# KleistLab/ADAPTed

Hardware: AMD Instinct MI355X
Metric: reads/sec (adapter+polyA detect), RNA004 200k-sample reads (higher is better)
Workload: dtype f32 samples/statistics, f64 cumulative sums + LLR trace

## Files before the change

adapted_amd/csrc/adapted_hip.hip:

```cpp
#include <hip/hip_runtime.h>

#include <cmath>
#include <cstdio>
#include <cstring>
#include <cstdlib>
#include <string>
#include <vector>

#include "adapted_hip.h"
#include "handle.h"
#include "common.h"
__device__ unsigned long long g_dbg[ADP_NDBG] = {0};
__device__ unsigned long long g_bs_tally[ADP_NTALLY][8] = {{0}};
#include "llr_stream.h"
#include "n1_select.h"
#include "n1_fused.h"
#include "peaks.h"
#include "synth.h"
#include "validate.h"
#include "cand_stats2.h"
#include "series_pipe.h"
#include "cnn_topk.h"
#include "cnn_conv.h"
#include "cnn_conv_split.h"
// ... 483 lines not shown
        hipLaunchKernelGGL((k_n1_pick<1, N1_SAMPLE>), pg, dim3(256), 0, st, mbs, gh, gb, gc, mode, thr);
        { Scope s(h, !profile ? nullptr : (mode ? "k_n1_hist<1> mad" : "k_n1_hist<1> med"));
          hipLaunchKernelGGL((k_n1_hist<1, SIG>), hg, dim3(N1_THREADS), 0, st, dsig, n, m, T, minibatch, mode, mbs, gh, gb, gc, 1, N1_ALWAYS, cb, collect, 1, 8, tails); }
        hipLaunchKernelGGL((k_n1_pick<1, N1_FULL>), pg, dim3(256), 0, st, mbs, gh, gb, gc, mode, thr);
        hipLaunchKernelGGL(k_n1_finish, pg, dim3(1024), 0, st, mbs, cb, gc, gb, mode, thr);
        hipLaunchKernelGGL((k_n1_hist<0, SIG>), hg, dim3(N1_THREADS), 0, st, dsig, n, m, T, minibatch, mode, mbs, gh, gb, gc, 1, N1_IF_BAD, cb, 0, 1, 8, tails);
        hipLaunchKernelGGL((k_n1_pick<0, N1_FALLBACK>), pg, dim3(256), 0, st, mbs, gh, gb, gc, mode, thr);
        hipLaunchKernelGGL((k_n1_hist<1, SIG>), hg, dim3(N1_THREADS), 0, st, dsig, n, m, T, minibatch, mode, mbs, gh, gb, gc, 1, N1_IF_BAD, cb, 0, 1, 8, tails);
        hipLaunchKernelGGL((k_n1_pick<1, N1_FALLBACK>), pg, dim3(256), 0, st, mbs, gh, gb, gc, mode, thr);
        { Scope s(h, !profile ? nullptr : (mode ? "k_n1_hist<2> mad" : "k_n1_hist<2> med"));
          hipLaunchKernelGGL((k_n1_hist<2, SIG>), hg, dim3(N1_THREADS), 0, st, dsig, n, m, T, minibatch, mode, mbs, gh, gb, gc, 1, N1_IF_NOT_DONE, cb, 0, 1, 8, tails); }
        hipLaunchKernelGGL((k_n1_pick<2, N1_FULL>), pg, dim3(256), 0, st, mbs, gh, gb, gc, mode, thr);
    }
    return 0;
}

struct PhaseSync {
    hipEvent_t wait[3] = {nullptr, nullptr, nullptr};
    hipEvent_t done[3] = {nullptr, nullptr, nullptr};
};

static __device__ __host__ inline SigF32 sig_from(const SigF32 &s, size_t r0, int m) { return SigF32{s.base + r0 * (size_t)m}; }
static __device__ __host__ inline SigI16 sig_from(const SigI16 &s, size_t r0, int m) { return SigI16{s.base + r0 * (size_t)m, s.scale + r0, s.offset + r0, s.full_len + r0}; }
static inline SigIdx sig_subset(const SigF32 &s, const int32_t *sel) { return SigIdx{s.base, sel}; }
static inline SigIdxI16 sig_subset(const SigI16 &s, const int32_t *sel) { return SigIdxI16{s.base, s.scale, s.offset, s.full_len, sel}; }

static void launch_cumsum(adp_handle *h, int n)
{
    const int split = env_int("ADP_CUMSUM_GATHER", 1) != 0;
    hipLaunchKernelGGL(k_cumsum, dim3((n + 63) / 64), dim3(64), 0, h->stream, h->down.as<float>(), h->nvalid.as<int32_t>(), h->Lp, n,
                       h->nck, h->ck.as<double2>(), h->tail.as<double2>(), split);
    if (split)
        hipLaunchKernelGGL(k_cumsum_gather, dim3((n + 63) / 64), dim3(64), 0, h->stream, h->down.as<float>(), h->nvalid.as<int32_t>(), h->Lp, n,
                           h->nck, h->ck.as<double2>(), h->tail.as<double2>());
}

static void launch_polya_peak(adp_handle *h, int n, int mbsize, const double *pkv)
{
    const int grid = n < h->pslots ? n : h->pslots;
    hipLaunchKernelGGL(k_polya_peak, dim3(grid), dim3(64), (size_t)(((h->Lp / 2 + 1) + 8) / 16 + 2) * 4, h->stream, h->trace.as<double>(), h->nvalid.as<int32_t>(), h->Lp,
                       h->bmax.as<double>(), h->bmin.as<double>(), h->nsum, h->adapter_idx.as<int32_t>(), n, mbsize, h->mbs.as<MbState>(),
                       h->pk.as<int32_t>(), h->mk.as<uint32_t>(), h->polya_idx.as<int32_t>(), h->npk.as<int32_t>(), pkv, env_int("ADP_PK_PREFIX", PK_PREFIX));
}

template <class SIG>
static int llr_enqueue(adp_handle *h, SIG dsig, const int32_t *dlen, int n, int m, int minibatch, int flags,
                       adp_row *rows_dev, int rows_kind , int32_t *mb_status_dev, double *mb_params_dev,
                       int upto, const PhaseSync *ps)
{
    int rc = 0;
    const int n_mb = (n + minibatch - 1) / minibatch;
    h->last_n = n; h->last_nmb = n_mb;
    ALLOCCHK(h->mbs.ensure((size_t)n_mb * sizeof(MbState)) || h->ghist.ensure((size_t)n_mb * N1_BINS * 4) || h->gbelow.ensure((size_t)n_mb * 8) || h->gcnt.ensure((size_t)n_mb * 8 * N1_NCNT));
    rc = alloc_all(h, n, true);
    if (rc) return rc;
    hipStream_t st = h->stream;
#ifdef ADP_ABLATE
    sync_ablate(h);
#endif
    if (ps && ps->wait[0]) HIPCHK(hipStreamWaitEvent(st, ps->wait[0], 0));
    MbState *mbs = h->mbs.as<MbState>();
    HIPCHK(hipMemsetAsync(mbs, 0, (size_t)n_mb * sizeof(MbState), st));
    HIPCHK(hipMemsetAsync(h->ghist.p, 0, (size_t)n_mb * N1_BINS * 4, st));
    HIPCHK(hipMemsetAsync(h->gbelow.p, 0, (size_t)n_mb * 8, st));
    HIPCHK(hipMemsetAsync(h->gcnt.p, 0, (size_t)n_mb * 8 * N1_NCNT, st));
    const int T = h->T;
    bool sp_forked = false, sp_done = false;
    if (h->L <= 0) {
        hipLaunchKernelGGL(k_mb_set_status, dim3((n_mb + 255) / 256), dim3(256), 0, st, mbs, n_mb, ADP_MB_EMPTY_TRACE);
        if (ps) for (int k = 0; k < 2; k++) { if (k && ps->wait[k]) HIPCHK(hipStreamWaitEvent(st, ps->wait[k], 0)); if (ps->done[k]) HIPCHK(hipEventRecord(ps->done[k], st)); }
    } else {
        const int32_t *tails = (flags & ADP_TAILS_NAN) ? dlen : nullptr;
        rc = launch_n1(h, dsig, n, m, T, minibatch, n_mb, true, tails);
        if (rc) return rc;
        const bool sp_fused = upto >= 8 && (flags & ADP_WITH_START_PEAK) && h->layout == ADP_LAYOUT_MINIBATCH &&
                              h->cfg.sp_downscale_factor == h->ds && h->off % h->ds == 0 && T > h->off && env_int("ADP_SP_FUSED", 1) != 0;
        if (sp_fused) {
            ALLOCCHK(h->sphead.ensure((size_t)n * sizeof(SpHead)));
            Scope s(h, "k_sp_head");
            hipLaunchKernelGGL(k_sp_head<SIG>, dim3(n), dim3(64), (size_t)64 * h->cfg.sp_downscale_factor * 4, st, dsig, dlen, n, m, h->cfg, h->off, h->sphead.as<SpHead>());
        }
        if (upto >= 2 && sp_fused) {
            { Scope s(h, "k_norm_pool");
              auto kern = (h->ds == 10 && std::is_same<SIG, SigF32>::value && env_int("ADP_NP_PREFETCH", 1)) ? k_norm_pool<SIG, true, 5> : k_norm_pool<SIG, true, 0>;
              hipLaunchKernelGGL(kern, dim3(n), dim3(256), (size_t)NP_TILE * h->ds * 4, st, dsig, m, T, h->off, h->ds, h->L, h->Lp,
                                 minibatch, mbs, h->down.as<float>(), h->nvalid.as<int32_t>(), (const int64_t *)nullptr,
                                 dlen, (flags & ADP_TAILS_NAN) ? 1 : 0, h->sphead.as<SpHead>(), (float)h->cfg.open_pore_pa); }
            const int cov0 = h->off / h->ds, cov1 = cov0 + (T - h->off) / h->ds;
            Scope s(h, "k_sp_tail");
            hipLaunchKernelGGL(k_sp_tail<SIG>, dim3(n), dim3(64), (size_t)64 * h->cfg.sp_downscale_factor * 4, st, dsig, dlen, n, m, h->cfg, cov0, cov1,
                               (const SpHead *)h->sphead.as<SpHead>(), h->sp.as<SpOut>());
            sp_done = true;
        } else if (upto >= 2) {
            Scope s(h, "k_norm_pool");
            const int64_t *rng = nullptr;
            if (h->layout == ADP_LAYOUT_SINGLE_READ) {
                ALLOCCHK(h->rng0.ensure((size_t)n * 16));
                std::vector<int64_t> hr((size_t)2 * n);
                for (int i = 0; i < n; i++) { hr[2 * i] = 0; hr[2 * i + 1] = T; }
                HIPCHK(hipMemcpyAsync(h->rng0.p, hr.data(), (size_t)n * 16, hipMemcpyHostToDevice, st));
                HIPCHK(hipStreamSynchronize(st));
                rng = h->rng0.as<int64_t>();
            }
            auto kern = (h->ds == 10 && !rng && std::is_same<SIG, SigF32>::value && env_int("ADP_NP_PREFETCH", 1)) ? k_norm_pool<SIG, false, 5> : k_norm_pool<SIG, false, 0>;
            hipLaunchKernelGGL(kern, dim3(n), dim3(256), (size_t)NP_TILE * h->ds * 4, st, dsig, m, T, h->off, h->ds, h->L, h->Lp,
                               minibatch, mbs, h->down.as<float>(), h->nvalid.as<int32_t>(), rng,
                               dlen, (flags & ADP_TAILS_NAN) ? 1 : 0, (SpHead *)nullptr, 0.f);
        }
        if (upto >= 2)
            hipLaunchKernelGGL(k_check_empty, dim3((n + 255) / 256), dim3(256), 0, st, h->nvalid.as<int32_t>(), n, minibatch, mbs);
        if (ps && ps->done[0]) HIPCHK(hipEventRecord(ps->done[0], st));
        if (upto >= 8 && (flags & ADP_WITH_START_PEAK) && !sp_fused) {
            HIPCHK(hipEventRecord(h->ev_fork, st));
            HIPCHK(hipStreamWaitEvent(h->stream2, h->ev_fork, 0));
            { Scope s(h, "k_start_peak", h->stream2);
              hipLaunchKernelGGL(k_start_peak<SIG>, dim3(n), dim3(64), (size_t)64 * h->cfg.sp_downscale_factor * 4, h->stream2, dsig, dlen, n, m, h->cfg, h->sp.as<SpOut>()); }
            HIPCHK(hipEventRecord(h->ev_join, h->stream2));
            sp_forked = true;
        }
        if (ps && ps->wait[1]) HIPCHK(hipStreamWaitEvent(st, ps->wait[1], 0));
        if (upto >= 3) {
            Scope s(h, "k_cumsum");
            launch_cumsum(h, n);
        }
        if (upto >= 4) {
            Scope s(h, "k_gains<1>");
            hipLaunchKernelGGL(k_gains<1>, dim3((n + GAINS_WPB - 1) / GAINS_WPB), dim3(64 * GAINS_WPB), 0, st, h->down.as<float>(), h->nvalid.as<int32_t>(), h->Lp, h->nck,
                               h->ck.as<double2>(), h->tail.as<double2>(), h->adapter_idx.as<int32_t>(), minibatch, mbs,
                               h->trace.as<double>(), h->bmax.as<double>(), h->bmin.as<double>(), h->nsum, h->t1.as<int2>(), 0, h->pk.as<int32_t>(), h->npk.as<int32_t>(), h->Lp / 2 + 1, h->gstat.as<double>(), n, h->oh1);
        }
        if (upto >= 5) {
            Scope s(h, "k_adapter_peak");
            hipLaunchKernelGGL(k_adapter_peak, dim3(n), dim3(64), 0, st, h->trace.as<double>(), h->nvalid.as<int32_t>(), h->Lp,
                               h->bmax.as<double>(), h->bmin.as<double>(), h->nsum, h->t1.as<int2>(), minibatch, mbs,
                               h->cfg.adapter_peak_prominence, h->cfg.adapter_peak_rel_height,
                               h->cfg.adapter_peak_width / h->ds, h->adapter_idx.as<int32_t>(), h->gstat.as<double>());
        }
        double *pkvp = (env_int("ADP_PK_VALUES", 1) && h->pkv.cap >= (size_t)n * (h->Lp / 2 + 1) * 8) ? h->pkv.as<double>() : nullptr;
        if (upto >= 6) {
            Scope s(h, "k_gains<2>");
            hipLaunchKernelGGL(k_gains<2>, dim3((n + GAINS_WPB - 1) / GAINS_WPB), dim3(64 * GAINS_WPB), 0, st, h->down.as<float>(), h->nvalid.as<int32_t>(), h->Lp, h->nck,
                               h->ck.as<double2>(), h->tail.as<double2>(), h->adapter_idx.as<int32_t>(), minibatch, mbs,
                               h->trace.as<double>(), h->bmax.as<double>(), h->bmin.as<double>(), h->nsum, h->t1.as<int2>(), 0, h->pk.as<int32_t>(), h->npk.as<int32_t>(), h->Lp / 2 + 1, h->gstat.as<double>(), n, 5, pkvp);
        }
        if (upto >= 7) {
            Scope s(h, "k_polya_peak");
            launch_polya_peak(h, n, minibatch, pkvp);
        }
        if (ps && ps->done[1]) HIPCHK(hipEventRecord(ps->done[1], st));
    }
    if (upto >= 8) {
        if (ps && ps->wait[2]) HIPCHK(hipStreamWaitEvent(st, ps->wait[2], 0));
        if (h->L > 0)
            hipLaunchKernelGGL(k_llr_bounds, dim3((n + 255) / 256), dim3(256), 0, st, h->adapter_idx.as<int32_t>(),
                               h->polya_idx.as<int32_t>(), n, h->ds, h->pos_off, h->bounds.as<int64_t>(), h->topk_none.as<int8_t>(), h->layout == ADP_LAYOUT_SINGLE_READ ? 1 : 0);
        rc = launch_validate(h, dsig, dlen, n, m, 1, minibatch, true);
        if (rc) return rc;
        if (flags & ADP_WITH_START_PEAK) {
            if (sp_forked) HIPCHK(hipStreamWaitEvent(st, h->ev_join, 0));
            else if (!sp_done) {
                Scope s(h, "k_start_peak");
                hipLaunchKernelGGL(k_start_peak<SIG>, dim3(n), dim3(64), (size_t)64 * h->cfg.sp_downscale_factor * 4, st, dsig, dlen, n, m, h->cfg, h->sp.as<SpOut>());
            }
            hipLaunchKernelGGL(k_sp_decorate, dim3((n + 255) / 256), dim3(256), 0, st, h->sp.as<SpOut>(), h->rows.as<adp_row>(), n, 0,
                               (const int32_t *)nullptr);
        }
        if (rows_dev)
            HIPCHK(hipMemcpyAsync(rows_dev, h->rows.p, (size_t)n * sizeof(adp_row), (hipMemcpyKind)rows_kind, st));
    }
    if (mb_status_dev)
        hipLaunchKernelGGL(k_mb_status_out, dim3((n_mb + 255) / 256), dim3(256), 0, st, mbs, n_mb, mb_status_dev);
    if (mb_params_dev)
        hipLaunchKernelGGL(k_mb_params_out, dim3((n_mb + 255) / 256), dim3(256), 0, st, mbs, n_mb, mb_params_dev);
    if (ps && ps->done[2]) HIPCHK(hipEventRecord(ps->done[2], st));
    HIPCHK(hipGetLastError());
    return ADP_OK;
}

static bool trunc_wanted(int flags, const adp_row *rows) { return (flags & ADP_FLAG_TRUNCATED) && rows; }
static int trunc_supported(const adp_handle *h)
{
    const adp_cfg &c = h->cfg;
    const int W = c.median_shift_window;
    if (!c.mvs_detect_check) { g_err = "ADP_FLAG_TRUNCATED needs mvs_detect_check (its tests are the MVS check's)"; return ADP_ERR_UNSUPPORTED; }
    if (c.mvs_detect_overwrite) { g_err = "ADP_FLAG_TRUNCATED does not go with mvs_detect_overwrite"; return ADP_ERR_UNSUPPORTED; }
    if (h->layout == ADP_LAYOUT_SINGLE_READ) { g_err = "ADP_FLAG_TRUNCATED does not go with the single-read layout"; return ADP_ERR_UNSUPPORTED; }
    if (W > PT_WMAX) { g_err = "ADP_FLAG_TRUNCATED: median_shift_window is longer than the tail test holds in LDS (4096)"; return ADP_ERR_UNSUPPORTED; }
// ... 690 lines not shown
{
    hipLaunchKernelGGL(k_sp_decorate, dim3((n + 255) / 256), dim3(256), 0, h->stream, sp, rows, n, 0, (const int32_t *)nullptr);
}
template <class SIG>
static int cnn_enqueue(adp_handle *h, SIG dsig, const int32_t *dlen, int n_reads, int m, int minibatch, adp_row *rows_dst,
                       int rows_kind, int64_t *bounds_dst, int bounds_kind, SpOut *sp_out = nullptr)
{
    const int off = h->cfg.min_obs_adapter, ds = h->cfg.downscale_factor;
    const int Lc = (m - off + ds - 1) / ds, L1 = (Lc - 1) / 3 + 1, Lo = 3 * L1 - 2;
    ALLOCCHK(h->cnn_x.ensure((size_t)n_reads * Lc * 4) || h->cnn_sc.ensure((size_t)n_reads * 2 * Lo * 4));
    hipStream_t st = h->stream;
    int rc = alloc_all(h, n_reads, false);
    if (rc) return rc;
    const size_t sp_lds = (size_t)64 * h->cfg.sp_downscale_factor * 4;
    const bool sp_fused = sp_out && cnn_sp_fused(h);
    SpHead *sp_head = nullptr;
    if (sp_fused) {
        ALLOCCHK(h->sphead.ensure((size_t)n_reads * sizeof(SpHead)));
        sp_head = h->sphead.as<SpHead>();
        Scope s(h, "k_sp_head");
        hipLaunchKernelGGL(k_sp_head<SIG>, dim3(n_reads), dim3(64), sp_lds, st, dsig, dlen, n_reads, m, h->cfg, off, sp_head);
    }
    rc = launch_cnn_prepare(h, dsig, n_reads, m, off, ds, Lc, h->cnn_x.as<float>(), sp_head);
    if (rc) return rc;
    if (sp_fused) {
        const int cov0 = off / ds, cov1 = cov0 + (m - off) / ds;
        Scope s(h, "k_sp_tail");
        hipLaunchKernelGGL(k_sp_tail<SIG>, dim3(n_reads), dim3(64), sp_lds, st, dsig, dlen, n_reads, m, h->cfg, cov0, cov1, (const SpHead *)sp_head, sp_out);
    } else if (sp_out) {
        HIPCHK(hipEventRecord(h->ev_fork, st));
        HIPCHK(hipStreamWaitEvent(h->stream2, h->ev_fork, 0));
        { Scope s(h, "k_start_peak", h->stream2);
          hipLaunchKernelGGL(k_start_peak<SIG>, dim3(n_reads), dim3(64), sp_lds, h->stream2, dsig, dlen, n_reads, m, h->cfg, sp_out); }
        HIPCHK(hipEventRecord(h->ev_join, h->stream2));
    }
    struct SpJoin { hipStream_t side; bool armed; ~SpJoin() { if (armed) (void)hipStreamSynchronize(side); } } sp_join{h->stream2, sp_out && !sp_fused};
    rc = cnn_forward_dev(h, h->cnn_x.as<float>(), n_reads, Lc, h->cnn_sc.as<float>());
    if (rc) return rc;
    int kk = 1;
    rc = cnn_predict_dev(h, h->cnn_sc.as<float>(), n_reads, minibatch, Lo, &kk);
    if (rc) return rc;
    if (bounds_dst) HIPCHK(hipMemcpyAsync(bounds_dst, h->bounds.p, (size_t)n_reads * (1 + kk) * 8, (hipMemcpyKind)bounds_kind, st));
    HIPCHK(hipMemsetAsync(h->topk_none.p, 0, (size_t)n_reads, st));
    rc = launch_validate(h, dsig, dlen, n_reads, m, kk, n_reads, false);
    if (rc) return rc;
    if (sp_out) {
        if (!sp_fused) { HIPCHK(hipStreamWaitEvent(st, h->ev_join, 0)); sp_join.armed = false; }
        cnn_sp_decorate(h, sp_out, h->rows.as<adp_row>(), n_reads);
    }
    if (rows_dst) HIPCHK(hipMemcpyAsync(rows_dst, h->rows.p, (size_t)n_reads * sizeof(adp_row), (hipMemcpyKind)rows_kind, st));
    HIPCHK(hipGetLastError());
    return ADP_OK;
}

extern "C++" {
__global__ void k_refine_out(const MbState *mbs, const int32_t *nvalid, const int32_t *polya_idx, const int64_t *ranges, int n,
                             int ds, int64_t *out, int32_t *status)
{
    int r = blockIdx.x * blockDim.x + threadIdx.x;
    if (r >= n) return;
    int st = 0;
    if (mbs[r].status == ADP_MB_MAD_ZERO) st = ADP_F_EXC_MAD_ZERO;
    else if (nvalid[r] <= 0) st = ADP_F_EXC_EMPTY_TRACE;
    int p = polya_idx[r];
    out[r] = (st == 0 && p > 0) ? (int64_t)p * ds + ranges[2 * r] : 0;
    status[r] = st;
}

template <class SIG>
static int refine_chain(adp_handle *h, SIG dsig, const int32_t *dlen, int n, int m, const int64_t *drng, int64_t *dout, int32_t *dstat)
{
    hipStream_t st = h->stream;
    ALLOCCHK(h->mbs.ensure((size_t)n * sizeof(MbState)) || h->ghist.ensure((size_t)n * N1_BINS * 4) || h->gbelow.ensure((size_t)n * 8) || h->gcnt.ensure((size_t)n * 8 * N1_NCNT));
    MbState *mbs = h->mbs.as<MbState>();
    HIPCHK(hipMemsetAsync(mbs, 0, (size_t)n * sizeof(MbState), st));
    HIPCHK(hipMemsetAsync(h->ghist.p, 0, (size_t)n * N1_BINS * 4, st));
    HIPCHK(hipMemsetAsync(h->gbelow.p, 0, (size_t)n * 8, st));
    HIPCHK(hipMemsetAsync(h->adapter_idx.p, 0, (size_t)n * 4, st));
    HIPCHK(hipMemsetAsync(h->gcnt.p, 0, (size_t)n * 8 * N1_NCNT, st));
    { Scope s(h, "k_n1 (refine)");
      int rc = launch_n1(h, dsig, n, m, h->T, 1, n, false);
      if (rc) return rc; }
    { Scope s(h, "k_norm_pool (refine)");
      hipLaunchKernelGGL(k_norm_pool<SIG>, dim3(n), dim3(256), (size_t)NP_TILE * h->ds * 4, st, dsig, m, h->T, h->off, h->ds, h->L, h->Lp, 1, mbs,
                         h->down.as<float>(), h->nvalid.as<int32_t>(), drng, dlen); }
    { Scope s(h, "k_gains (refine)");
      launch_cumsum(h, n);
      hipLaunchKernelGGL(k_gains<1>, dim3((n + GAINS_WPB - 1) / GAINS_WPB), dim3(64 * GAINS_WPB), 0, st, h->down.as<float>(), h->nvalid.as<int32_t>(), h->Lp, h->nck,
                         h->ck.as<double2>(), h->tail.as<double2>(), h->adapter_idx.as<int32_t>(), 1, mbs, h->trace.as<double>(),
                         h->bmax.as<double>(), h->bmin.as<double>(), h->nsum, h->t1.as<int2>(), 1, h->pk.as<int32_t>(), h->npk.as<int32_t>(), h->Lp / 2 + 1, (double *)nullptr, n, 5); }
    { Scope s(h, "k_polya_peak (refine)");
      launch_polya_peak(h, n, 1, nullptr);
      hipLaunchKernelGGL(k_refine_out, dim3((n + 255) / 256), dim3(256), 0, st, mbs, h->nvalid.as<int32_t>(), h->polya_idx.as<int32_t>(),
                         drng, n, h->ds, dout, dstat); }
    return 0;
}
}

static bool cnn_fallback_wanted(const adp_handle *h, int flags, const adp_row *rows)
{
    return (flags & ADP_CNN_FALLBACK) && h->cfg.fallback_to_llr_short_reads && rows;
}
static int cnn_fallback_select(adp_handle *h, const int32_t *dlen, int n, const adp_row *rows, const int64_t *bounds, int bstride)
{
    ALLOCCHK(h->fb_sel.ensure((size_t)n * 4));
    Scope s(h, "k_cnn_fb_select");
    hipLaunchKernelGGL(k_cnn_fb_select, dim3(1), dim3(SEL_THREADS), 0, h->stream, rows, bounds, bstride, dlen, n, 2ll * h->cfg.max_obs_adapter,
                       h->fb_sel.as<int32_t>(), h->op_used.as<unsigned int>() + 2);
    return 0;
}

template <class SIG>
static int cnn_fallback_run(adp_handle *h, SIG dsig, const int32_t *dlen, int m, adp_row *rows, const int64_t *bounds, int bstride, int n_sel)
{
    hipStream_t st = h->stream;
    int rc = alloc_all(h, n_sel, true);
    if (rc) return rc;
    const size_t N = (size_t)n_sel;
    int64_t *drng, *dout, *db2; int32_t *dstat, *dlen_sub; int8_t *topk; adp_row *rows2;
    RCCHK(sub_carve(h, [&](Carve &c) {
        drng = c.take<int64_t>(2 * N); dout = c.take<int64_t>(N); db2 = c.take<int64_t>(2 * N);
        dstat = c.take<int32_t>(N); dlen_sub = c.take<int32_t>(N); topk = c.take<int8_t>(N); rows2 = c.take<adp_row>(N);
    }));
    unsigned int *counts = phase_counts(h, OPW_FB);
    const int32_t *sel = h->fb_sel.as<int32_t>();
    const auto sig = sig_subset(dsig, sel);
    HIPCHK(hipMemsetAsync(counts, 0, 8, st));
    HIPCHK(hipMemsetAsync(topk, 0, N, st));
    { Scope s(h, "k_cnn_fb_gather");
      hipLaunchKernelGGL(k_cnn_fb_gather, dim3((n_sel + 255) / 256), dim3(256), 0, st, sel, n_sel, 0, bounds, bstride, dlen, dlen_sub, drng,
                         (const int64_t *)nullptr, (const int32_t *)nullptr, (int64_t *)nullptr); }
    rc = refine_chain(h, sig, dlen_sub, n_sel, m, drng, dout, dstat);
    if (rc) return rc;
    { Scope s(h, "k_cnn_fb_gather");
      hipLaunchKernelGGL(k_cnn_fb_gather, dim3((n_sel + 255) / 256), dim3(256), 0, st, sel, n_sel, 1, bounds, bstride, dlen, dlen_sub, drng,
                         (const int64_t *)dout, (const int32_t *)dstat, db2); }
    const ValBufs vb{db2, topk, rows2};
    rc = launch_validate(h, sig, dlen_sub, n_sel, m, 1, n_sel, false, &vb);
    if (rc) return rc;
    { Scope s(h, "k_cnn_fb_merge");
      hipLaunchKernelGGL(k_cnn_fb_merge, dim3(n_sel), dim3(64), 0, st, sel, n_sel, (const int64_t *)dout, (const int32_t *)dstat,
                         (const adp_row *)rows2, rows, counts); }
    HIPCHK(hipGetLastError());
    return 0;
}

static bool cnn_second_wanted(int flags, const adp_row *rows) { return (flags & ADP_CNN_SECOND_LLR) && rows; }
static bool cnn_sp_wanted(int flags, const adp_row *rows) { return (flags & ADP_WITH_START_PEAK) && rows; }
static int cnn_second_select(adp_handle *h, int n, const adp_row *rows)
{
    ALLOCCHK(h->so_sel.ensure((size_t)n * 4));
    Scope s(h, "k_cnn_so_select");
    hipLaunchKernelGGL(k_cnn_so_select, dim3(1), dim3(SEL_THREADS), 0, h->stream, rows, n, h->so_sel.as<int32_t>(), h->op_used.as<unsigned int>() + 3);
    return 0;
}

template <class SIG>
static int cnn_second_run(adp_handle *h, SIG dsig, const int32_t *dlen, int n, int m, int minibatch, int flags, adp_row *rows, int n_so)
{
    hipStream_t st = h->stream;
    const int tails = std::is_same<SIG, SigF32>::value ? (flags & ADP_TAILS_NAN) : ADP_TAILS_NAN;
    int rc = llr_enqueue(h, dsig, dlen, n, m, minibatch, tails, nullptr, 0, nullptr, nullptr, 7, nullptr);
    if (rc) return rc;
    const size_t R = (size_t)n, N = (size_t)n_so;
    int64_t *ball, *b2; int32_t *dlen_sub; int8_t *tall, *tsub; adp_row *rows2;
    RCCHK(sub_carve(h, [&](Carve &c) {
        ball = c.take<int64_t>(2 * R); tall = c.take<int8_t>(R);
        b2 = c.take<int64_t>(2 * N); dlen_sub = c.take<int32_t>(N); tsub = c.take<int8_t>(N); rows2 = c.take<adp_row>(N);
// ... 432 lines not shown
```

adapted_amd/csrc/common.h:

```cpp
#pragma once
#define ADP_NDBG 80
#define ADP_NTALLY 256
#include <hip/hip_runtime.h>
#include <stdint.h>

#include "adapted_hip.h"

#define LDS __attribute__((address_space(3)))
#define GLB __attribute__((address_space(1)))
#define WAVE 64
#define CK 16
#define TRACE_TILE 1024
#define SUMBLK 64

#ifdef ADP_ABLATE
extern __device__ int g_ablate;
#define ABLATED(bits) ((g_ablate & (bits)) != 0)
#else
#define ABLATED(bits) false
#endif

struct MbState {
    unsigned long long n_valid;
    unsigned long long krem;
// ... 179 lines not shown

static __device__ __forceinline__ uint32_t f2key(float f)
{
    const uint32_t u = __float_as_uint(f);
    return u ^ ((uint32_t)((int32_t)u >> 31) | 0x80000000u);
}
static __device__ __forceinline__ float key2f(uint32_t k)
{
    uint32_t u = (k & 0x80000000u) ? (k & 0x7fffffffu) : ~k;
    return __uint_as_float(u);
}
static __device__ __forceinline__ uint64_t d2key(double d)
{
    const uint64_t u = (uint64_t)__double_as_longlong(d);
    return u ^ ((uint64_t)((int64_t)u >> 63) | 0x8000000000000000ULL);
}
static __device__ __forceinline__ double key2d(uint64_t k)
{
    const uint64_t u = (k & 0x8000000000000000ULL) ? (k & 0x7fffffffffffffffULL) : ~k;
    return __longlong_as_double((long long)u);
}

template <class T>
static __device__ __forceinline__ T wave_sum(T v)
{
#pragma unroll
    for (int o = 32; o > 0; o >>= 1) v += __shfl_xor(v, o);
    return v;
}
template <class T>
static __device__ __forceinline__ T wave_max(T v)
{
#pragma unroll
    for (int o = 32; o > 0; o >>= 1) { T w = __shfl_xor(v, o); v = w > v ? w : v; }
    return v;
}
template <class T>
static __device__ __forceinline__ T wave_min(T v)
{
#pragma unroll
    for (int o = 32; o > 0; o >>= 1) { T w = __shfl_xor(v, o); v = w < v ? w : v; }
    return v;
}
static __device__ __forceinline__ int wave_scan_incl(int v)
{
#pragma unroll
    for (int o = 1; o < 64; o <<= 1) { int w = __shfl_up(v, o); if (lane_id() >= o) v += w; }
    return v;
}

#define SEL_THREADS 1024
static __device__ __forceinline__ void sel_step(bool take, int r, int32_t *__restrict__ sel, int &total)
{
    __shared__ __attribute__((aligned(16))) int s_wave[SEL_THREADS / 64];
    const int ln = lane_id(), w = threadIdx.x >> 6;
    const unsigned long long mk = __ballot(take);
    if (ln == 0) s_wave[w] = __popcll(mk);
    __syncthreads();
    int before = 0, step = 0;
    for (int i = 0; i < SEL_THREADS / 64; i++) { const int c = s_wave[i]; if (i < w) before += c; step += c; }
    if (take) sel[total + before + __popcll(mk & ((1ull << ln) - 1ull))] = r;
    total += step;
    __syncthreads();
}

template <class F>
static __device__ __forceinline__ float pw_leaf_f32(int n, F get)
{
    if (n < 8) {
        float res = 0.f;
        for (int i = 0; i < n; i++) res += get(i);
        return res;
    }
    float r0 = get(0), r1 = get(1), r2 = get(2), r3 = get(3), r4 = get(4), r5 = get(5), r6 = get(6), r7 = get(7);
    int i;
    for (i = 8; i < n - (n % 8); i += 8) {
        r0 += get(i); r1 += get(i + 1); r2 += get(i + 2); r3 += get(i + 3);
        r4 += get(i + 4); r5 += get(i + 5); r6 += get(i + 6); r7 += get(i + 7);
    }
    float res = ((r0 + r1) + (r2 + r3)) + ((r4 + r5) + (r6 + r7));
    for (; i < n; i++) res += get(i);
    return res;
}
```

adapted_amd/csrc/llr_stream.h:

```cpp
#pragma once
#include <type_traits>
#include "common.h"
#include "log_cr.h"
#include "wave_stats.h"

#define NP_TILE 512
struct SpHead {
    int32_t valid, max_idx, a2, e0;
    float mx;
    int32_t op_end;
    int32_t op_head, op_body, hit;
    int32_t pad;
};

template <class SIG, bool SP = false, int NQ = 0>
__global__ void __launch_bounds__(256) k_norm_pool(SIG sig, int m, int T, int off, int ds, int L, int Lp,
                                                   int mbsize, const MbState *__restrict__ mbs,
                                                   float *__restrict__ down, int32_t *__restrict__ nvalid,
                                                   const int64_t *__restrict__ ranges, const int32_t *__restrict__ full_len,
                                                   int tails_nan = 0, SpHead *__restrict__ sp_head = nullptr, float sp_thr = 0.f)
{
    extern __shared__ __attribute__((aligned(16))) float tile[];
    __shared__ int s_nan;
    __shared__ __attribute__((aligned(16))) int s_sp[2];
    const int r = blockIdx.x;
    const MbState st = mbs[r / mbsize];
    if (st.status != ADP_MB_OK) { if (threadIdx.x == 0) nvalid[r] = 0; return; }
    const float med = st.med, mad = st.mad, lo = st.lo, hi = st.hi;
    int Lseg = T - off;
    if (ranges) {
        long long a = ranges[2 * r], b = ranges[2 * r + 1];
        long long lim = full_len[r] < T ? full_len[r] : T;
        if (b > lim) b = lim;
        off = (int)a;
        Lseg = (int)(b > a ? b - a : 0);
        L = (Lseg + ds - 1) / ds;
        if (L > Lp) L = Lp;
    }
    const typename SIG::Row row = sig.row(r, m) + off;
    if (threadIdx.x == 0) s_nan = 0;
    int my_nan = 0;
    float sp_mx = 0.f;
    int sp_a2 = 0, sp_e0 = 0, sp_op_end = 0, sp_hit = 0x7fffffff, sp_op = 0x7fffffff;
    const int sp_full = (T - off) / ds;
    const int sp_pb0 = off / ds;
    if (SP) {
        const SpHead hd = sp_head[r];
        sp_mx = hd.mx; sp_a2 = hd.valid ? hd.a2 : 0; sp_e0 = hd.valid ? hd.e0 : 0; sp_op_end = hd.op_end;
        if (threadIdx.x < 2) s_sp[threadIdx.x] = 0x7fffffff;
    }
    int L_ok = L;
    if (tails_nan && !ranges) {
        long long lv = (long long)full_len[r] - off;
        if (lv < Lseg) { if (lv < 0) lv = 0; L_ok = (int)(lv / ds); }
    }
    const int tile_n = NP_TILE * ds;
    const bool vec = row.vec_ok() && ((tile_n & 3) == 0);
    const bool fast_div = fdiv_ok(mad);
    const float rmad = 1.0f / mad;
    auto norm1 = [&](float c) {
        c = c < lo ? lo : c;
        c = c > hi ? hi : c;
        return fast_div ? fdiv_shared(c - med, mad, rmad) : (c - med) / mad;
    };
    const bool use_pf = NQ > 0 && vec && tile_n / 4 == NQ * 256;
    float4 pre[NQ > 0 ? NQ : 1];
    auto fetch = [&](int tb_) {
        const int base_ = tb_ * ds;
        const typename SIG::Row rowb = row + base_;
#pragma unroll
        for (int u = 0; u < (NQ > 0 ? NQ : 1); u++) {
            const int q = threadIdx.x + u * 256;
            const int idx = base_ + 4 * q;
            float4 v = make_float4(0.f, 0.f, 0.f, 0.f);
            if (idx + 3 < Lseg) v = rowb.f4s(q);
            else {
                if (idx < Lseg) v.x = row[idx];
                if (idx + 1 < Lseg) v.y = row[idx + 1];
                if (idx + 2 < Lseg) v.z = row[idx + 2];
            }
            pre[u] = v;
        }
    };
    if (use_pf && L_ok > 0 && L > 0) fetch(0);
    for (int tb = 0; tb < L; tb += NP_TILE) {
        const int base = tb * ds;
        if (tb >= L_ok) {
            for (int jj = threadIdx.x; jj < NP_TILE; jj += 256) if (tb + jj < L) { down[(size_t)r * Lp + tb + jj] = __builtin_nanf(""); my_nan++; }
            continue;
        }
        __syncthreads();
        if (use_pf) {
#pragma unroll
            for (int u = 0; u < (NQ > 0 ? NQ : 1); u++) {
                const int q = threadIdx.x + u * 256;
                const int idx = base + 4 * q;
                float4 v = pre[u];
                if (!SP) {
                    v.x = idx < Lseg ? norm1(v.x) : 0.f; v.y = idx + 1 < Lseg ? norm1(v.y) : 0.f;
                    v.z = idx + 2 < Lseg ? norm1(v.z) : 0.f; v.w = idx + 3 < Lseg ? norm1(v.w) : 0.f;
                }
                reinterpret_cast<float4 *>(tile)[q] = v;
            }
        } else if (vec) {
            const typename SIG::Row rowb = row + base;
            for (int q = threadIdx.x; q < tile_n / 4; q += 256) {
                const int idx = base + 4 * q;
                float4 v = make_float4(0.f, 0.f, 0.f, 0.f);
                if (SP) {
                    const float padv = -__builtin_inff();
                    v = make_float4(padv, padv, padv, padv);
                    if (idx + 3 < Lseg) v = rowb.f4s(q);
                    else {
                        if (idx < Lseg) v.x = row[idx];
                        if (idx + 1 < Lseg) v.y = row[idx + 1];
                        if (idx + 2 < Lseg) v.z = row[idx + 2];
                    }
                } else if (idx + 3 < Lseg) { v = rowb.f4s(q); v.x = norm1(v.x); v.y = norm1(v.y); v.z = norm1(v.z); v.w = norm1(v.w); }
                else {
                    if (idx < Lseg) v.x = norm1(row[idx]);
                    if (idx + 1 < Lseg) v.y = norm1(row[idx + 1]);
                    if (idx + 2 < Lseg) v.z = norm1(row[idx + 2]);
                }
                reinterpret_cast<float4 *>(tile)[q] = v;
            }
        } else {
            for (int i = threadIdx.x; i < tile_n; i += 256) {
                int idx = base + i;
                if (SP) tile[i] = (idx < Lseg) ? row[idx] : -__builtin_inff();
                else tile[i] = (idx < Lseg) ? norm1(row[idx]) : 0.0f;
            }
        }
        __syncthreads();
        if (use_pf) { const int nx = tb + NP_TILE; if (nx < L && nx < L_ok) fetch(nx); }
        for (int jj = threadIdx.x; jj < NP_TILE; jj += 256) {
            const int j = tb + jj;
            if (j < L) {
                const float *p = tile + jj * ds;
                float s;
                if (SP) {
                    const int nin = Lseg - j * ds;
                    if (nin >= ds) s = pw_leaf_f32(ds, [&](int k) { return norm1(p[k]); });
                    else s = pw_leaf_f32(ds, [&](int k) { return k < nin ? norm1(p[k]) : 0.0f; });
                    if (j < sp_full) {
                        const int g = sp_pb0 + j;
                        if (g >= sp_a2 && g < sp_e0) {
                            const float v = pw_leaf_f32(ds, [&](int k) { return p[k]; }) / (float)ds;
                            if (v > sp_mx && g < sp_hit) sp_hit = g;
                        }
                        const int i0 = off + j * ds;
                        if (i0 < sp_op_end && sp_op == 0x7fffffff) {
                            for (int k = 0; k < ds; k++) if (i0 + k < sp_op_end && p[k] > sp_thr) { sp_op = i0 + k; break; }
                        }
                    }
                } else s = pw_leaf_f32(ds, [&](int k) { return p[k]; });
                float pooled = s / (float)ds;
                down[(size_t)r * Lp + j] = pooled;
                if (pooled != pooled) my_nan++;
            }
        }
    }
    if (SP) {
        sp_hit = wave_min(sp_hit); sp_op = wave_min(sp_op);
        if (lane_id() == 0) { if (sp_hit != 0x7fffffff) atomicMin(&s_sp[0], sp_hit); if (sp_op != 0x7fffffff) atomicMin(&s_sp[1], sp_op); }
    }
    my_nan = wave_sum(my_nan);
    if (lane_id() == 0 && my_nan) atomicAdd(&s_nan, my_nan);
    __syncthreads();
    if (threadIdx.x == 0) {
        nvalid[r] = L - s_nan;
        if (SP) { sp_head[r].hit = s_sp[0]; sp_head[r].op_body = s_sp[1]; }
    }
}

static __device__ __forceinline__ bool csum_uniform(int n) { return wave_max(n) - wave_min(n) < 8 * CK; }
__global__ void __launch_bounds__(64) k_cumsum(const float *__restrict__ down, const int32_t *__restrict__ nvalid, int Lp, int n_reads,
                                               int nck, double2 *__restrict__ ck, double2 *__restrict__ tail, int split)
{
    const int r = blockIdx.x * 64 + threadIdx.x;
    const int n = r < n_reads ? nvalid[r] : 0;
    if (split && csum_uniform(n)) return;
    if (r >= n_reads) return;
    const float *s = down + (size_t)r * Lp;
    double2 *c = ck + (size_t)r * nck;
    double a = 0.0, b = 0.0;
    double2 t = make_double2(0.0, 0.0);
    const float4 *s4 = reinterpret_cast<const float4 *>(s);
    auto block = [&](int j0, const float4 (&q)[4]) {
        c[j0 / CK] = make_double2(a, b);
        const float v[16] = {q[0].x, q[0].y, q[0].z, q[0].w, q[1].x, q[1].y, q[1].z, q[1].w, q[2].x, q[2].y, q[2].z, q[2].w, q[3].x, q[3].y, q[3].z, q[3].w};
        if (j0 + CK < n) {
#pragma unroll
            for (int u = 0; u < CK; u++) { const double x = (double)v[u]; a += x; b += x * x; }
        } else {
#pragma unroll
            for (int u = 0; u < CK; u++) {
                const int j = j0 + u;
                if (j < n) {
                    if (j == n - 1) t = make_double2(a, b);
                    double x = (double)v[u];
                    a += x;
                    b += x * x;
                }
            }
        }
    };
    constexpr int PFL = 2;
    float4 q[PFL][2][4];
    const int last_line = Lp / (2 * CK) - 1;
    auto ldl = [&](int line, float4 (&qq)[2][4]) {
        const float4 *p4 = s4 + (line < last_line ? line : last_line) * (2 * CK / 4);
#pragma unroll
        for (int e = 0; e < 8; e++) qq[e >> 2][e & 3] = p4[e];
    };
#pragma unroll
    for (int d = 0; d < PFL; d++) ldl(d, q[d]);
    for (int j0 = 0; j0 < n; j0 += PFL * 2 * CK) {
        const int line = j0 / (2 * CK);
#pragma unroll
        for (int d = 0; d < PFL; d++) {
            const int j1 = j0 + d * 2 * CK;
            if (d == 0 || j1 < n) block(j1, q[d][0]);
            if (j1 + CK < n) block(j1 + CK, q[d][1]);
            ldl(line + PFL + d, q[d]);
        }
    }
    tail[r] = t;
}

#define CSUM_Q 8
typedef double csum_d2 __attribute__((ext_vector_type(2)));
__global__ void __launch_bounds__(64) k_cumsum_gather(const float *__restrict__ down, const int32_t *__restrict__ nvalid, int Lp, int n_reads,
                                                      int nck, double2 *__restrict__ ck, double2 *__restrict__ tail)
{
    __shared__ __attribute__((aligned(16))) csum_d2 cks_[64 * (CSUM_Q + 1)];
    LDS csum_d2 *cks = (LDS csum_d2 *)cks_;
    const int ln = threadIdx.x, r0 = blockIdx.x * 64;
    const int r = r0 + ln;
    const int n = r < n_reads ? nvalid[r] : 0;
    if (!csum_uniform(n)) return;
    const int nmax = wave_max(n);
    const float *s = down + (size_t)(r < n_reads ? r : n_reads - 1) * Lp;
    double a = 0.0, b = 0.0;
    double2 t = make_double2(0.0, 0.0);
// ... 306 lines not shown
```

Before: 1.080 million.

## Specialize norm-pool kernel for compile-time downscale factor with unrolled pooling

```diff
diff --git a/adapted_amd/csrc/adapted_hip.hip b/adapted_amd/csrc/adapted_hip.hip
--- a/adapted_amd/csrc/adapted_hip.hip
+++ b/adapted_amd/csrc/adapted_hip.hip
@@ -589,7 +589,8 @@
         }
         if (upto >= 2 && sp_fused) {
             { Scope s(h, "k_norm_pool");
-              auto kern = (h->ds == 10 && std::is_same<SIG, SigF32>::value && env_int("ADP_NP_PREFETCH", 1)) ? k_norm_pool<SIG, true, 5> : k_norm_pool<SIG, true, 0>;
+              auto kern = h->ds != 10 ? k_norm_pool<SIG, true, 0, 0> :
+                          (std::is_same<SIG, SigF32>::value && env_int("ADP_NP_PREFETCH", 1)) ? k_norm_pool<SIG, true, 5, 10> : k_norm_pool<SIG, true, 0, 10>;
               hipLaunchKernelGGL(kern, dim3(n), dim3(256), (size_t)NP_TILE * h->ds * 4, st, dsig, m, T, h->off, h->ds, h->L, h->Lp,
                                  minibatch, mbs, h->down.as<float>(), h->nvalid.as<int32_t>(), (const int64_t *)nullptr,
                                  dlen, (flags & ADP_TAILS_NAN) ? 1 : 0, h->sphead.as<SpHead>(), (float)h->cfg.open_pore_pa); }
@@ -609,7 +610,8 @@
                 HIPCHK(hipStreamSynchronize(st));
                 rng = h->rng0.as<int64_t>();
             }
-            auto kern = (h->ds == 10 && !rng && std::is_same<SIG, SigF32>::value && env_int("ADP_NP_PREFETCH", 1)) ? k_norm_pool<SIG, false, 5> : k_norm_pool<SIG, false, 0>;
+            auto kern = h->ds != 10 ? k_norm_pool<SIG, false, 0, 0> :
+                        (!rng && std::is_same<SIG, SigF32>::value && env_int("ADP_NP_PREFETCH", 1)) ? k_norm_pool<SIG, false, 5, 10> : k_norm_pool<SIG, false, 0, 10>;
             hipLaunchKernelGGL(kern, dim3(n), dim3(256), (size_t)NP_TILE * h->ds * 4, st, dsig, m, T, h->off, h->ds, h->L, h->Lp,
                                minibatch, mbs, h->down.as<float>(), h->nvalid.as<int32_t>(), rng,
                                dlen, (flags & ADP_TAILS_NAN) ? 1 : 0, (SpHead *)nullptr, 0.f);
@@ -1466,8 +1468,9 @@
       int rc = launch_n1(h, dsig, n, m, h->T, 1, n, false);
       if (rc) return rc; }
     { Scope s(h, "k_norm_pool (refine)");
-      hipLaunchKernelGGL(k_norm_pool<SIG>, dim3(n), dim3(256), (size_t)NP_TILE * h->ds * 4, st, dsig, m, h->T, h->off, h->ds, h->L, h->Lp, 1, mbs,
-                         h->down.as<float>(), h->nvalid.as<int32_t>(), drng, dlen); }
+      auto kern = h->ds == 10 ? k_norm_pool<SIG, false, 0, 10> : k_norm_pool<SIG, false, 0, 0>;
+      hipLaunchKernelGGL(kern, dim3(n), dim3(256), (size_t)NP_TILE * h->ds * 4, st, dsig, m, h->T, h->off, h->ds, h->L, h->Lp, 1, mbs,
+                         h->down.as<float>(), h->nvalid.as<int32_t>(), drng, dlen, 0, (SpHead *)nullptr, 0.f); }
     { Scope s(h, "k_gains (refine)");
       launch_cumsum(h, n);
       hipLaunchKernelGGL(k_gains<1>, dim3((n + GAINS_WPB - 1) / GAINS_WPB), dim3(64 * GAINS_WPB), 0, st, h->down.as<float>(), h->nvalid.as<int32_t>(), h->Lp, h->nck,
diff --git a/adapted_amd/csrc/common.h b/adapted_amd/csrc/common.h
--- a/adapted_amd/csrc/common.h
+++ b/adapted_amd/csrc/common.h
@@ -285,3 +285,28 @@
     for (; i < n; i++) res += get(i);
     return res;
 }
+
+template <int N, class F>
+static __device__ __forceinline__ float pw_leaf_f32(F get)
+{
+    static_assert(N >= 1 && N <= 128, "one leaf of numpy's pairwise sum");
+    if constexpr (N < 8) {
+        float res = 0.f;
+#pragma unroll
+        for (int i = 0; i < N; i++) res += get(i);
+        return res;
+    } else {
+        float r[8];
+#pragma unroll
+        for (int u = 0; u < 8; u++) r[u] = get(u);
+#pragma unroll
+        for (int i = 8; i < N - (N % 8); i += 8) {
+#pragma unroll
+            for (int u = 0; u < 8; u++) r[u] += get(i + u);
+        }
+        float res = ((r[0] + r[1]) + (r[2] + r[3])) + ((r[4] + r[5]) + (r[6] + r[7]));
+#pragma unroll
+        for (int i = N - (N % 8); i < N; i++) res += get(i);
+        return res;
+    }
+}
diff --git a/adapted_amd/csrc/llr_stream.h b/adapted_amd/csrc/llr_stream.h
--- a/adapted_amd/csrc/llr_stream.h
+++ b/adapted_amd/csrc/llr_stream.h
@@ -13,8 +13,19 @@
     int32_t pad;
 };
 
-template <class SIG, bool SP = false, int NQ = 0>
-__global__ void __launch_bounds__(256) k_norm_pool(SIG sig, int m, int T, int off, int ds, int L, int Lp,
+template <bool FD, bool FC>
+static __device__ __forceinline__ float np_norm1(float c, float lo, float hi, float med, float mad, float rmad)
+{
+    if (FC) c = __builtin_amdgcn_fmed3f(c, lo, hi);
+    else {
+        c = c < lo ? lo : c;
+        c = c > hi ? hi : c;
+    }
+    return FD ? fdiv_shared(c - med, mad, rmad) : (c - med) / mad;
+}
+
+template <class SIG, bool SP = false, int NQ = 0, int DS = 0>
+__global__ void __launch_bounds__(256) k_norm_pool(SIG sig, int m, int T, int off, int ds_rt, int L, int Lp,
                                                    int mbsize, const MbState *__restrict__ mbs,
                                                    float *__restrict__ down, int32_t *__restrict__ nvalid,
                                                    const int64_t *__restrict__ ranges, const int32_t *__restrict__ full_len,
@@ -22,7 +33,10 @@
 {
     extern __shared__ __attribute__((aligned(16))) float tile[];
     __shared__ int s_nan;
+    __shared__ int s_nan_tile;
     __shared__ __attribute__((aligned(16))) int s_sp[2];
+    static_assert(DS % 2 == 0 && DS <= 14, "the straight pooling body reads 8-byte pieces and adds numpy's tail behind ONE round of the accumulators");
+    const int ds = DS > 0 ? DS : ds_rt;
     const int r = blockIdx.x;
     const MbState st = mbs[r / mbsize];
     if (st.status != ADP_MB_OK) { if (threadIdx.x == 0) nvalid[r] = 0; return; }
@@ -38,7 +52,7 @@
         if (L > Lp) L = Lp;
     }
     const typename SIG::Row row = sig.row(r, m) + off;
-    if (threadIdx.x == 0) s_nan = 0;
+    if (threadIdx.x == 0) { s_nan = 0; s_nan_tile = -1; }
     int my_nan = 0;
     float sp_mx = 0.f;
     int sp_a2 = 0, sp_e0 = 0, sp_op_end = 0, sp_hit = 0x7fffffff, sp_op = 0x7fffffff;
@@ -58,31 +72,34 @@
     const bool vec = row.vec_ok() && ((tile_n & 3) == 0);
     const bool fast_div = fdiv_ok(mad);
     const float rmad = 1.0f / mad;
+    const bool clip_med3 = lo <= hi;
+    const bool use_pf = NQ > 0 && vec && tile_n / 4 == NQ * 256;
+    auto tiles = [&](auto fd_c, auto pf_c) {
+    constexpr bool FD = decltype(fd_c)::value;
+    constexpr bool PF = decltype(pf_c)::value;
     auto norm1 = [&](float c) {
-        c = c < lo ? lo : c;
-        c = c > hi ? hi : c;
-        return fast_div ? fdiv_shared(c - med, mad, rmad) : (c - med) / mad;
-    };
-    const bool use_pf = NQ > 0 && vec && tile_n / 4 == NQ * 256;
+        if (DS > 0) return np_norm1<FD, false>(c, lo, hi, med, mad, rmad);
+        return fast_div ? np_norm1<true, false>(c, lo, hi, med, mad, rmad) : np_norm1<false, false>(c, lo, hi, med, mad, rmad);
+    };
     float4 pre[NQ > 0 ? NQ : 1];
     auto fetch = [&](int tb_) {
-        const int base_ = tb_ * ds;
-        const typename SIG::Row rowb = row + base_;
+        const int t4 = 4 * threadIdx.x;
 #pragma unroll
         for (int u = 0; u < (NQ > 0 ? NQ : 1); u++) {
-            const int q = threadIdx.x + u * 256;
-            const int idx = base_ + 4 * q;
+            const int base_ = tb_ * ds + u * 1024;
+            const typename SIG::Row rowu = row + base_;
+            const int left = Lseg - base_;
             float4 v = make_float4(0.f, 0.f, 0.f, 0.f);
-            if (idx + 3 < Lseg) v = rowb.f4s(q);
+            if (t4 + 3 < left) v = rowu.f4s(threadIdx.x);
             else {
-                if (idx < Lseg) v.x = row[idx];
-                if (idx + 1 < Lseg) v.y = row[idx + 1];
-                if (idx + 2 < Lseg) v.z = row[idx + 2];
+                if (t4 < left) v.x = rowu[t4];
+                if (t4 + 1 < left) v.y = rowu[t4 + 1];
+                if (t4 + 2 < left) v.z = rowu[t4 + 2];
             }
             pre[u] = v;
         }
     };
-    if (use_pf && L_ok > 0 && L > 0) fetch(0);
+    if (PF && L_ok > 0 && L > 0) fetch(0);
     for (int tb = 0; tb < L; tb += NP_TILE) {
         const int base = tb * ds;
         if (tb >= L_ok) {
@@ -90,12 +107,16 @@
             continue;
         }
         __syncthreads();
-        if (use_pf) {
+        bool saw_nan = false;
+        auto look4 = [&](const float4 &v) { if (SP && DS > 0) { const float t = (v.x + v.y) + (v.z + v.w); saw_nan |= t != t; } };
+        if (PF) {
 #pragma unroll
             for (int u = 0; u < (NQ > 0 ? NQ : 1); u++) {
                 const int q = threadIdx.x + u * 256;
                 const int idx = base + 4 * q;
                 float4 v = pre[u];
+                if (SP && DS > 0) asm volatile("" : "+v"(v.x), "+v"(v.y), "+v"(v.z), "+v"(v.w));
+                look4(v);
                 if (!SP) {
                     v.x = idx < Lseg ? norm1(v.x) : 0.f; v.y = idx + 1 < Lseg ? norm1(v.y) : 0.f;
                     v.z = idx + 2 < Lseg ? norm1(v.z) : 0.f; v.w = idx + 3 < Lseg ? norm1(v.w) : 0.f;
@@ -116,6 +137,7 @@
                         if (idx + 1 < Lseg) v.y = row[idx + 1];
                         if (idx + 2 < Lseg) v.z = row[idx + 2];
                     }
+                    look4(v);
                 } else if (idx + 3 < Lseg) { v = rowb.f4s(q); v.x = norm1(v.x); v.y = norm1(v.y); v.z = norm1(v.z); v.w = norm1(v.w); }
                 else {
                     if (idx < Lseg) v.x = norm1(row[idx]);
@@ -127,12 +149,77 @@
         } else {
             for (int i = threadIdx.x; i < tile_n; i += 256) {
                 int idx = base + i;
-                if (SP) tile[i] = (idx < Lseg) ? row[idx] : -__builtin_inff();
+                if (SP) { const float c = (idx < Lseg) ? row[idx] : -__builtin_inff(); tile[i] = c; if (DS > 0) saw_nan |= c != c; }
                 else tile[i] = (idx < Lseg) ? norm1(row[idx]) : 0.0f;
             }
         }
+        if (SP && DS > 0 && saw_nan) s_nan_tile = tb;
         __syncthreads();
-        if (use_pf) { const int nx = tb + NP_TILE; if (nx < L && nx < L_ok) fetch(nx); }
+        const bool tile_nan = SP && DS > 0 && __builtin_amdgcn_readfirstlane(s_nan_tile) == tb;
+        if (PF) { const int nx = tb + NP_TILE; if (nx < L && nx < L_ok) fetch(nx); }
+        if constexpr (DS > 0) {
+            auto read_block = [&](int h, float (&xb)[DS]) {
+                const float2 *p2 = reinterpret_cast<const float2 *>(tile + (threadIdx.x + 256 * h) * DS);
+#pragma unroll
+                for (int k = 0; k < DS / 2; k++) { const float2 v = p2[k]; xb[2 * k] = v.x; xb[2 * k + 1] = v.y; }
+            };
+            const float fds = (float)DS, rds = 1.0f / fds;
+            const bool ds_fast = fdiv_ok(fds);
+            auto mean = [&](float s) {
+                const float pooled = ds_fast ? fdiv_shared(s, fds, rds) : s / fds;
+                if (pooled != pooled) my_nan++;
+                return pooled;
+            };
+            float *const dn = down + (size_t)r * Lp + tb + threadIdx.x;
+            auto riders = [&](int j, const float (&xb)[DS]) {
+                const int g = sp_pb0 + j;
+                if (g >= sp_a2 && g < sp_e0) {
+                    const float v = pw_leaf_f32<DS>([&](int k) { return xb[k]; }) / fds;
+                    if (v > sp_mx && g < sp_hit) sp_hit = g;
+                }
+                const int i0 = off + j * DS;
+                if (i0 < sp_op_end && sp_op == 0x7fffffff) {
+#pragma unroll
+                    for (int k = DS - 1; k >= 0; k--) if (i0 + k < sp_op_end && xb[k] > sp_thr) sp_op = i0 + k;
+                }
+            };
+            const bool interior = tb + NP_TILE <= L && (tb + NP_TILE) * DS <= Lseg && (!SP || tb + NP_TILE <= sp_full);
+            if (interior) {
+                auto body = [&](auto fc_c) {
+                    constexpr bool FC = decltype(fc_c)::value;
+#pragma unroll
+                    for (int h = 0; h < 2; h++) {
+                        const int j = tb + threadIdx.x + 256 * h;
+                        float xb[DS];
+                        read_block(h, xb);
+                        float s;
+                        if (SP) {
+                            s = pw_leaf_f32<DS>([&](int k) { return np_norm1<FD, FC>(xb[k], lo, hi, med, mad, rmad); });
+                            riders(j, xb);
+                        } else s = pw_leaf_f32<DS>([&](int k) { return xb[k]; });
+                        dn[256 * h] = mean(s);
+                    }
+                };
+                if (SP && clip_med3 && !tile_nan) body(std::true_type{});
+                else body(std::false_type{});
+            } else {
+#pragma unroll
+                for (int h = 0; h < 2; h++) {
+                    const int j = tb + threadIdx.x + 256 * h;
+                    float xb[DS];
+                    read_block(h, xb);
+                    if (j < L) {
+                        float s;
+                        if (SP) {
+                            const int nin = Lseg - j * DS;
+                            s = pw_leaf_f32<DS>([&](int k) { return k < nin ? np_norm1<FD, false>(xb[k], lo, hi, med, mad, rmad) : 0.0f; });
+                            if (j < sp_full) riders(j, xb);
+                        } else s = pw_leaf_f32<DS>([&](int k) { return xb[k]; });
+                        dn[256 * h] = mean(s);
+                    }
+                }
+            }
+        } else {
         for (int jj = threadIdx.x; jj < NP_TILE; jj += 256) {
             const int j = tb + jj;
             if (j < L) {
@@ -159,7 +246,15 @@
                 if (pooled != pooled) my_nan++;
             }
         }
-    }
+        }
+    }
+    };
+    auto tiles_fd = [&](auto pf_c) {
+        if (DS > 0 && !fast_div) tiles(std::false_type{}, pf_c);
+        else tiles(std::true_type{}, pf_c);
+    };
+    if constexpr (NQ > 0) { if (use_pf) tiles_fd(std::true_type{}); else tiles_fd(std::false_type{}); }
+    else tiles_fd(std::false_type{});
     if (SP) {
         sp_hit = wave_min(sp_hit); sp_op = wave_min(sp_op);
         if (lane_id() == 0) { if (sp_hit != 0x7fffffff) atomicMin(&s_sp[0], sp_hit); if (sp_op != 0x7fffffff) atomicMin(&s_sp[1], sp_op); }
```

Result: slower. 1.053 million (-2.5%).
